# KhaledSharif/yolo-from-scratch

Hardware: NVIDIA B200
Metric: decode+global-NMS + CIoU-loss fwd+bwd throughput @640^2 bs64 nc1 (higher is better)
Workload: dtype f32

## Files before the change

yolo-from-scratch_b200/csrc/yb_nms_graph.cu:

```cuda
#include "yb_common.cuh"
#include "yb_sort.cuh"
#include <cuda_fp16.h>
#include <atomic>
#include <mutex>
#include <vector>

namespace yb {

constexpr int kTile = 32;
constexpr int kSub = 8;
constexpr int kSubs = kTile / kSub;
constexpr uint32_t kNoSub = 0xffffffffu;
constexpr int kGatherThreads = 256;
constexpr int kEdgeThreads = 256;
#ifndef YB_EDGE_CTAS
#define YB_EDGE_CTAS 4
#endif
constexpr int kEdgeCtasPerSM = YB_EDGE_CTAS;
constexpr int kResolveThreads = 1024;

enum { G_PLAIN = 0, G_TRICK = 1, G_CLASS = 2 };

struct GImg {
    int M, mode, exact, overflow;
    int n_tiles;
    u32 n_edges;
    float s_off, t2;
    unsigned long long n_evals;
    unsigned long long n_cands;
};

struct GArgs {
    const float4* boxes;
    const float* scores;
    const int64_t* classes;
    const int* counts;
    int B, cap, tcap, scap;
    float thr;
    int thr_fast_ok;
    float t3;
    u32 k16x2;
    int hexp;
    long long trick_max_numel;
    u32 *k0, *v0;
    int n_score_chunks;
    u32* order;
    u32* rinv;
    u32* pos;
    float4* sboxes;
    u32* skey;
    u32* scls;
    int* iflags;
    int n_chunks;
    u32 resolve_smem_words;
    float4* tstat;
    float4* sstat;
    GImg* info;
    u32* ticket;
    u32 ticket_init;
    uint2* edges;
    u64 edges_per_img;
    int64_t* keep;
    int* n_keep;
};

template <int NT>
__device__ __forceinline__ float block_reduce_minmax(float v, bool is_max, float* s32, int lane, int warp) {
#pragma unroll
    for (int o = 16; o > 0; o >>= 1) {
        const float n = __shfl_xor_sync(0xffffffffu, v, o);
        v = is_max ? fmaxf(v, n) : fminf(v, n);
    }
    __syncthreads();
    if (lane == 0) s32[warp] = v;
    __syncthreads();
    float r = s32[0];
    for (int w = 1; w < NT / 32; ++w) r = is_max ? fmaxf(r, s32[w]) : fminf(r, s32[w]);
    return r;
}

__device__ __forceinline__ unsigned short hilbert_lut_entry(int state, u32 x, u32 y) {
    if (state & 1) { x = 15u - x; y = 15u - y; }
    if (state & 2) { const u32 t = x; x = y; y = t; }
    u32 d = 0, c = 0, sw = 0;
#pragma unroll
    for (u32 s = 8u; s > 0u; s >>= 1) {
        const u32 rx = (x & s) ? 1u : 0u, ry = (y & s) ? 1u : 0u;
        d += s * s * ((3u * rx) ^ ry);
        if (ry == 0u) {
            if (rx == 1u) { x = 15u - x; y = 15u - y; c ^= 1u; }
            const u32 t = x; x = y; y = t;
            sw ^= 1u;
        }
    }
    return (unsigned short)(d | ((((u32)state & 1u) ^ c) << 8) | (((((u32)state >> 1) & 1u) ^ sw) << 9));
}
__device__ __forceinline__ u32 hilbert8(const unsigned short* lut, u32 x, u32 y) {
    const u32 e = lut[((x >> 4) << 4) | (y >> 4)];
    const u32 e2 = lut[((e >> 8) << 8) | ((x & 15u) << 4) | (y & 15u)];
    return ((e & 255u) << 8) | (e2 & 255u);
}

__device__ __forceinline__ u32 area_bucket(const float4 q) {
    const float area = (q.z - q.x) * (q.w - q.y);
    const float lg = fminf(fmaxf(__log2f(area), -44.0f), 120.0f);
    return (u32)(int)floorf(lg * 0.6666667f + 32.0f) & 0x7fu;
}

constexpr int kKeyBits = 14;
struct KeyBits {
    int cls_shift, bkt_shift, bkt_drop, curve_drop;
    u32 bmin;
// ... 52 lines not shown
    const u32* ckey = a.k0 + off;
    const u32 key = ckey[p];
    const int c = p / kScoreChunk;
    u32 rank = (u32)(p - c * kScoreChunk);
    for (int o = 0; o * kScoreChunk < M; ++o) {
        if (o == c) continue;
        const u32* run = ckey + (size_t)o * kScoreChunk;
        const int len = min(kScoreChunk, M - o * kScoreChunk);
        int lo = 0, hi = len;
        while (lo < hi) {
            const int mid = (lo + hi) >> 1;
            const u32 k = run[mid];
            const bool before = o < c ? k <= key : k < key;
            if (before) lo = mid + 1; else hi = mid;
        }
        rank += (u32)lo;
    }
    const u32 idx = a.v0[off + p];
    a.order[off + rank] = idx;
    a.rinv[off + idx] = rank;
}

constexpr int kChunk = 26880;
constexpr int kSpThreads = 1024;
constexpr int kSpBatch = 4;

__host__ __device__ inline size_t spatial_smem_bytes(int ccap) {
    return ((size_t)1 << kKeyBits) * sizeof(u32) + 2 * (((size_t)ccap + 7) / 8 * 8) * sizeof(unsigned short) +
           1024 * sizeof(unsigned short);
}

__global__ void __launch_bounds__(kSpThreads) graph_spatial_kernel(const GArgs a) {
    extern __shared__ __align__(16) u32 s_dyn[];
    __shared__ float s_f[32];
    __shared__ int s_flag[32];
    __shared__ int s_maxcls[32];
    __shared__ int s_bmin[32], s_bmax[32];
    __shared__ u32 s_scan[32];
    constexpr int NT = kSpThreads;
    constexpr int NB = 1 << kKeyBits;

    const int chunk = blockIdx.x, b = blockIdx.y, tid = threadIdx.x, lane = tid & 31, warp = tid >> 5;
    const size_t off = (size_t)b * a.cap;
    {
        const int ccap0 = (min(a.cap, kChunk) + 7) & ~7;
        unsigned short* lut0 = reinterpret_cast<unsigned short*>(s_dyn + NB) + 2 * ccap0;
        lut0[tid] = hilbert_lut_entry(tid >> 8, (u32)(tid >> 4) & 15u, (u32)tid & 15u);
#pragma unroll
        for (int k = 0; k < NB / NT; ++k) s_dyn[k * NT + tid] = 0u;
    }
    int M = a.counts ? a.counts[b] : a.cap;
    M = M < 0 ? 0 : (M > a.cap ? a.cap : M);
    GImg* info = a.info + b;
    if (b == 0 && chunk == 0 && tid == 0) *a.ticket = a.ticket_init;
    const int c0 = chunk * kChunk;
    const int Mc = min(M - c0, kChunk);
    if (Mc <= 0) {
        if (tid == 0 && chunk == 0) {
            GImg z = {0, G_PLAIN, 0, 0, 0, 0u, 0.0f, -1.0f, 0ull, 0ull};
            *info = z;
            if (a.n_chunks == 1) a.iflags[b] = 0;
        }
        return;
    }
    const float4* boxes = a.boxes + off + c0;
    const int64_t* classes = a.classes ? a.classes + off + c0 : nullptr;
    const int ccap = (min(a.cap, kChunk) + 7) & ~7;
    u32* hist = s_dyn;
    unsigned short* keys = reinterpret_cast<unsigned short*>(s_dyn + NB);
    unsigned short* oidx = keys + ccap;
    unsigned short* lut = oidx + ccap;


    const int mode = !a.classes ? G_PLAIN : ((long long)M * 4 <= a.trick_max_numel ? G_TRICK : G_CLASS);
    float mx = -INFINITY, cmin = INFINITY, cmax = -INFINITY;
    int bad = 0, maxcls = 0, bmin = 127, bmax = 0;
    for (int i0 = tid; i0 < Mc; i0 += kSpBatch * NT) {
        float4 qv[kSpBatch];
        long long cv[kSpBatch];
#pragma unroll
        for (int u = 0; u < kSpBatch; ++u) {
            const int i = i0 + u * NT;
            if (i < Mc) {
                qv[u] = __ldg(boxes + i);
                cv[u] = classes ? __ldg(classes + i) : 0ll;
            }
        }
#pragma unroll
        for (int u = 0; u < kSpBatch; ++u) {
            if (i0 + u * NT >= Mc) break;
            const float4 q = qv[u];
            mx = fmaxf(mx, fmaxf(fmaxf(q.x, q.y), fmaxf(q.z, q.w)));
            const bool nan = (q.x != q.x) || (q.y != q.y) || (q.z != q.z) || (q.w != q.w);
            const float big = fmaxf(fmaxf(fabsf(q.x), fabsf(q.y)), fmaxf(fabsf(q.z), fabsf(q.w)));
            bad |= (nan ? 4 : 0) | ((nan || !(big <= 1e17f) || !(q.z >= q.x) || !(q.w >= q.y)) ? 1 : 0);
            const float cx = (q.x + q.z) * 0.5f, cy = (q.y + q.w) * 0.5f;
            cmin = fminf(cmin, fminf(cx, cy));
            cmax = fmaxf(cmax, fmaxf(cx, cy));
            const int bk = (int)area_bucket(q);
            bmin = min(bmin, bk);
            bmax = max(bmax, bk);
            if (classes) {
                const long long c = cv[u];
                bad |= (c < 0 || c >= 512) ? 2 : 0;
                maxcls = max(maxcls, (int)(c & 0x1ff));
            }
        }
// ... 127 lines not shown
    if (p >= M && p < ((M + kSub - 1) & ~(kSub - 1)))
        sbo[p] = make_float4(1e18f, 1e18f, 2e18f, 2e18f);
    if (p < M) {
        const u32 idx = a.pos[off + p];
        float4 q = boxes[idx];
        const float sc = a.scores[off + idx];
        u32 c = 0;
        if (classes) c = (u32)classes[idx];
        if (info.mode == G_TRICK) {
            const float o = (float)classes[idx] * info.s_off;
            q.x += o; q.y += o; q.z += o; q.w += o;
        }
        const u32 cls = (info.mode == G_CLASS) ? c : 0u;
        sbo[p] = q;
        a.skey[off + p] = desc_key(sc);
        if (info.mode == G_CLASS) a.scls[off + p] = cls;
        x1 = f2ord(q.x); y1 = f2ord(q.y); x2 = f2ord(q.z); y2 = f2ord(q.w);
        amin = amax = f2ord((q.z - q.x) * (q.w - q.y));
        c0 = c1 = cls;
    }
    u32 sx1 = x1, sy1 = y1, sx2 = x2, sy2 = y2, samin = amin, samax = amax;
#pragma unroll
    for (int o = 1; o < kSub; o <<= 1) {
        sx1 = min(sx1, __shfl_xor_sync(0xffffffffu, sx1, o));
        sy1 = min(sy1, __shfl_xor_sync(0xffffffffu, sy1, o));
        sx2 = max(sx2, __shfl_xor_sync(0xffffffffu, sx2, o));
        sy2 = max(sy2, __shfl_xor_sync(0xffffffffu, sy2, o));
        samin = min(samin, __shfl_xor_sync(0xffffffffu, samin, o));
        samax = max(samax, __shfl_xor_sync(0xffffffffu, samax, o));
    }
    if ((lane & (kSub - 1)) == 0) {
        float4* ss = a.sstat + (((size_t)b * a.tcap + t) * kSubs + (lane / kSub)) * 2;
        ss[0] = make_float4(ord2f(sx1), ord2f(sy1), ord2f(sx2), ord2f(sy2));
        ss[1] = make_float4(ord2f(samin), ord2f(samax), 0.0f, 0.0f);
    }
    const u32 tx1 = __reduce_min_sync(0xffffffffu, sx1), ty1 = __reduce_min_sync(0xffffffffu, sy1);
    const u32 tx2 = __reduce_max_sync(0xffffffffu, sx2), ty2 = __reduce_max_sync(0xffffffffu, sy2);
    const u32 tamin = __reduce_min_sync(0xffffffffu, samin), tamax = __reduce_max_sync(0xffffffffu, samax);
    c0 = __reduce_min_sync(0xffffffffu, c0);
    c1 = __reduce_max_sync(0xffffffffu, c1);
    if (lane == 0) {
        float4* ts = a.tstat + ((size_t)b * a.tcap + t) * 2;
        ts[0] = make_float4(ord2f(tx1), ord2f(ty1), ord2f(tx2), ord2f(ty2));
        ts[1] = make_float4(ord2f(tamin), ord2f(tamax), __uint_as_float(c0), __uint_as_float(c1));
    }
}

struct Rec16 {
    uint4 box;
    u32 area;
    u32 pad[3];
};
constexpr int kSlots = 8;
constexpr int kQueue = kTile + 8;
constexpr int kCand = 3 * kTile;
constexpr int kItems = kSlots * kTile + kSlots;
struct EdgeWarp {
    Rec16 row16[kTile + 1];
    Rec16 col16[kSlots * 4];
    u32 tl[kTile];
    u32 sub[kQueue];
    uint2 sbx[kQueue];
    u32 sar[kQueue];
    unsigned short irow[kItems];
    unsigned short icol[kItems];
    u32 cand[kCand];
    uint2 ebuf[2 * kTile];
};

__device__ __forceinline__ u32 pack2(const unsigned short lo, const unsigned short hi) { return (u32)lo | ((u32)hi << 16); }
__device__ __forceinline__ __half2 as_h2(const u32 v) { return *reinterpret_cast<const __half2*>(&v); }
__device__ __forceinline__ u32 as_u32(const __half2 v) { return *reinterpret_cast<const u32*>(&v); }
__device__ __forceinline__ unsigned short h_dn(const float v) { return __half_as_ushort(__float2half_rd(v)); }
__device__ __forceinline__ unsigned short h_up(const float v) { return __half_as_ushort(__float2half_ru(v)); }
__device__ __forceinline__ unsigned short h_rz(const float v) { return __half_as_ushort(__float2half_rz(v)); }
__device__ __forceinline__ bool h2_all_ge(const u32 a, const u32 b) {
    u32 r;
    asm("{\n\t.reg .pred p, q;\n\tsetp.ge.f16x2 p|q, %1, %2;\n\tand.pred p, p, q;\n\tselp.u32 %0, 1, 0, p;\n\t}" : "=r"(r) : "r"(a), "r"(b));
    return r != 0u;
}
__device__ __forceinline__ bool h2_any_ge0(const u32 a) {
    u32 r;
    asm("{\n\t.reg .pred p, q;\n\tsetp.ge.f16x2 p|q, %1, %2;\n\tor.pred p, p, q;\n\tselp.u32 %0, 1, 0, p;\n\t}" : "=r"(r) : "r"(a), "r"(0u));
    return r != 0u;
}
__device__ __forceinline__ u32 h2_ge0_bits(const u32 a) {
    u32 r;
    asm("{\n\t.reg .pred p, q;\n\t.reg .u32 t;\n\tsetp.ge.f16x2 p|q, %1, %2;\n\tselp.u32 %0, 1, 0, p;\n\tselp.u32 t, 2, 0, q;\n\tor.b32 %0, %0, t;\n\t}"
        : "=r"(r) : "r"(a), "r"(0u));
    return r;
}

struct Frame {
    float S, S2, nox, noy;
};
__device__ __forceinline__ unsigned short area16_down(const float4 q, const float S2) {
    const float a = __fmul_rd(__fmul_rd(__fsub_rd(q.z, q.x), __fsub_rd(q.w, q.y)), S2);
    return a >= 2.44140625e-4f ? h_rz(fminf(a, 32768.0f)) : (unsigned short)0xfb53u;
}

__device__ __forceinline__ void edge_flush(const GArgs& a, EdgeWarp& w, int b, uint2* __restrict__ edges, int& n_buf) {
    if (n_buf == 0) return;
    const int lane = threadIdx.x & 31;
    __syncwarp();
    u32 base = 0;
    if (lane == 0) base = atomicAdd(&a.info[b].n_edges, (u32)n_buf);
    base = __shfl_sync(0xffffffffu, base, 0);
    for (int k = lane; k < n_buf; k += 32) {
        const u64 idx = (u64)base + k;
        if (idx < a.edges_per_img) edges[idx] = w.ebuf[k];
    }
    __syncwarp();
    n_buf = 0;
// ... 100 lines not shown
                const int at = n_items + __popc(m & lt_mask);
                w.irow[at] = my_row;
                w.icol[at] = (unsigned short)(s * 4 * (int)sizeof(Rec16));
            }
            n_items += __popc(m);
        }
    }
    if (lane < kSlots) {
        w.irow[n_items + lane] = (unsigned short)(kTile * (int)sizeof(Rec16));
        w.icol[n_items + lane] = 0;
    }
    n_evals += (u32)n_items;
    __syncwarp();

    const __half2 K = as_h2(a.k16x2);
    const __half2 zero = as_h2(0u);
    const char* rowbase = reinterpret_cast<const char*>(w.row16);
    const char* colbase = reinterpret_cast<const char*>(w.col16) + j * sizeof(Rec16);
    const unsigned short* irow = w.irow + grp;
    const unsigned short* icol = w.icol + grp;
    for (int it = 0; it < n_items; it += kSlots) {
        const u32 ro = irow[it], co = icol[it];
        const Rec16* rr = reinterpret_cast<const Rec16*>(rowbase + ro);
        const Rec16* cc = reinterpret_cast<const Rec16*>(colbase + co);
        const uint4 R = rr->box, C = cc->box;
        const __half2 iw = __hmax2(__hsub2(__hmin2(as_h2(R.z), as_h2(C.z)), __hmax2(as_h2(R.x), as_h2(C.x))), zero);
        const __half2 ih = __hsub2(__hmin2(as_h2(R.w), as_h2(C.w)), __hmax2(as_h2(R.y), as_h2(C.y)));
        const __half2 sum = __hadd2(as_h2(rr->area), as_h2(cc->area));
        const u32 x = as_u32(__hfma2(__hmul2(iw, ih), K, __hneg2(sum)));
        if (!__any_sync(0xffffffffu, h2_any_ge0(x))) continue;
        const u32 i = ro / (u32)sizeof(Rec16);
        const u32 qp = sub[co / (u32)(4 * sizeof(Rec16))] * kSub + 2 * j;
        const u32 rp = (u32)I * kTile + i;
        u32 hit = ro < (u32)(kTile * sizeof(Rec16)) ? h2_ge0_bits(x) : 0u;
        if (qp <= rp) hit &= 2u;
        if (qp + 1u <= rp) hit = 0u;
        const unsigned m0 = __ballot_sync(0xffffffffu, hit != 0u);
        if (m0 == 0u) continue;
        if (hit) w.cand[n_cand + __popc(m0 & lt_mask)] = (i << 24) | (qp + (hit == 2u ? 1u : 0u));
        n_cand += __popc(m0);
        const unsigned m1 = __ballot_sync(0xffffffffu, hit == 3u);
        if (m1) {
            if (hit == 3u) w.cand[n_cand + __popc(m1 & lt_mask)] = (i << 24) | (qp + 1u);
            n_cand += __popc(m1);
        }
        if (n_cand >= kTile) {
            n_cands += (u32)n_cand;
            cand_process(a, w, M, class_mode, b, I, n_cand, n_buf);
        }
    }
    __syncwarp();
}

__global__ void __launch_bounds__(kEdgeThreads, kEdgeCtasPerSM) graph_edge_kernel(const GArgs a) {
    __shared__ __align__(16) EdgeWarp s_w[kEdgeThreads / 32];
    const int lane = threadIdx.x & 31;
    EdgeWarp& w = s_w[threadIdx.x >> 5];
    const unsigned lt_mask = (1u << lane) - 1u;
    int max_tiles = 0;
    for (int i = lane; i < a.B; i += 32) max_tiles = max(max_tiles, a.iflags[i] ? 0 : a.info[i].n_tiles);
    max_tiles = __reduce_max_sync(0xffffffffu, max_tiles);
    const u32 total = (u32)max_tiles * (u32)a.B;

    bool first = true;
    for (;;) {
        u32 ticket = blockIdx.x * (kEdgeThreads / 32) + (threadIdx.x >> 5);
        if (!first) {
            if (lane == 0) ticket = atomicAdd(a.ticket, 1u);
            ticket = __shfl_sync(0xffffffffu, ticket, 0);
        }
        first = false;
        if (ticket >= total) break;
        const int I = max_tiles - 1 - (int)(ticket / (u32)a.B), b = (int)(ticket % (u32)a.B);
        const float4* sb = a.sboxes + (size_t)b * a.scap;
        const float4* ts = a.tstat + (size_t)b * a.tcap * 2;
        const float4* ss = a.sstat + (size_t)b * a.tcap * kSubs * 2;
        const float4 ib = ts[I * 2], ia = ts[I * 2 + 1];
        const int rp = I * kTile + lane;
        const float4 rq = rp < a.scap ? sb[rp] : make_float4(0.f, 0.f, 0.f, 0.f);
        const int flagged = a.iflags[b];
        const GImg info = a.info[b];
        if (I >= info.n_tiles || flagged) continue;
        const int M = info.M;
        const float t2 = info.t2;
        const float t3 = a.t3;
        const bool class_mode = info.mode == G_CLASS;

        Frame f;
        {
            const float ext = fmaxf(ib.z - ib.x, ib.w - ib.y) * 0.5f;
            int k = a.hexp - ((int)((__float_as_uint(ext) >> 23) & 255u) - 127);
            k = max(-60, min(60, k));
            f.S = __int_as_float((127 + k) << 23);
            f.S2 = f.S * f.S;
            f.nox = -((ib.x + ib.z) * 0.5f) * f.S;
            f.noy = -((ib.y + ib.w) * 0.5f) * f.S;
        }
        const u32 icmin = __float_as_uint(ia.z), icmax = __float_as_uint(ia.w);

        const bool rvalid = rp < M;
        u32 r_lo = 0x63d063d0u, r_hi = 0xe3d0e3d0u, r_wh_t = 0x63d063d0u, r_ar = 0xe3d063d0u;
        __syncwarp();
        {
            Rec16& r16 = w.row16[lane];
            uint4 box = make_uint4(0x63d063d0u, 0x63d063d0u, 0xe3d0e3d0u, 0xe3d0e3d0u);
            u32 area = 0x3c003c00u;
            if (rvalid) {
                const unsigned short x1 = h_dn(__fmaf_rd(rq.x, f.S, f.nox)), y1 = h_dn(__fmaf_rd(rq.y, f.S, f.noy));
                const unsigned short x2 = h_up(__fmaf_ru(rq.z, f.S, f.nox)), y2 = h_up(__fmaf_ru(rq.w, f.S, f.noy));
                const unsigned short ar = area16_down(rq, f.S2);
                const float wd = __fsub_rd(rq.z, rq.x), hd = __fsub_rd(rq.w, rq.y);
                const unsigned short wt = h_rz(__fmul_rd(__fmul_rd(wd, f.S), t3)), ht = h_rz(__fmul_rd(__fmul_rd(hd, f.S), t3));
                const unsigned short at = h_rz(__fmul_rd(__fmul_rd(__fmul_rd(wd, hd), f.S2), t3));
                const unsigned short au = h_up(__fmul_ru(__fmul_ru(__fsub_ru(rq.z, rq.x), __fsub_ru(rq.w, rq.y)), f.S2)) ^ 0x8000u;
                r_lo = pack2(x1, y1);
                r_hi = pack2(x2, y2);
                r_wh_t = pack2(wt, ht);
                r_ar = pack2(at, au);
                box = make_uint4(pack2(x1, x1), pack2(y1, y1), pack2(x2, x2), pack2(y2, y2));
                area = pack2(ar, ar);
            }
            r16.box = box;
            r16.area = area;
            if (lane == 0) {
                Rec16& sen = w.row16[kTile];
                sen.box = make_uint4(0x63d063d0u, 0x63d063d0u, 0xe3d0e3d0u, 0xe3d0e3d0u);
                sen.area = 0x3c003c00u;
            }
        }
        __syncwarp();
        u32 n_evals = 0, n_cands = 0;
        int n_q = 0;
        int n_buf = 0;
        int n_cand = 0;

        constexpr int kCT = kChunk / kTile;
        int chunk_end = min(info.n_tiles, (I / kCT + 1) * kCT);
        for (int J0 = I;; J0 += 32) {
            if (J0 >= chunk_end && chunk_end < info.n_tiles) {
                J0 = chunk_end;
                chunk_end = min(info.n_tiles, chunk_end + kCT);
                if (class_mode) {
                    const int step = (chunk_end - J0 + 31) / 32;
                    const int Jp = J0 + lane * step;
                    const bool ge = Jp < chunk_end && __float_as_uint(ts[Jp * 2 + 1].w) >= icmin;
                    const unsigned m = __ballot_sync(0xffffffffu, ge);
                    const int first = m ? __ffs(m) - 1 : 32;
                    J0 += max(first - 1, 0) * step;
                }
            }
            const bool tail = J0 >= info.n_tiles;
            int n_t = 0;
            int n_tail = kSlots;
            if (tail) {
                if (n_q == 0) break;
                if (lane >= n_q && lane < kSlots) w.sub[lane] = kNoSub;
                n_tail = n_q;
                n_q = kSlots;
                __syncwarp();
            } else {
                const int Jl = J0 + lane;
                bool ok = Jl < chunk_end;
                float4 jb = make_float4(0.f, 0.f, 0.f, 0.f), ja = jb;
                if (ok) { jb = ts[Jl * 2]; ja = ts[Jl * 2 + 1]; }
                if (class_mode) {
                    const bool beyond = !ok || __float_as_uint(ja.z) > icmax;
                    ok = ok && !beyond && __float_as_uint(ja.w) >= icmin;
                    if (__ballot_sync(0xffffffffu, beyond) == 0xffffffffu) {
                        J0 = chunk_end - 32;
                        continue;
                    }
                }
                if (ok) {
                    ok = fminf(ib.z, jb.z) > fmaxf(ib.x, jb.x) && fminf(ib.w, jb.w) > fmaxf(ib.y, jb.y) &&
                         ia.y >= t2 * ja.x && ja.y >= t2 * ia.x;
                }
                const unsigned cand = __ballot_sync(0xffffffffu, ok);
                if (cand == 0u) continue;
                if (ok) w.tl[__popc(cand & lt_mask)] = (u32)Jl;
                __syncwarp();
                n_t = __popc(cand);
            }
            int t0 = 0;
            do {
                if (t0 < n_t) {
                    const int k = t0 + lane / kSubs;
                    bool sok = k < n_t;
                    u32 e = 0u;
                    float4 sbx = make_float4(0.f, 0.f, 0.f, 0.f), sar = sbx;
                    if (sok) {
                        e = w.tl[k] * kSubs + (u32)(lane & (kSubs - 1));
                        sok = (int)(e * kSub) < M;
                        if (sok) {
                            sbx = ss[e * 2]; sar = ss[e * 2 + 1];
                            sok = fminf(ib.z, sbx.z) > fmaxf(ib.x, sbx.x) && fminf(ib.w, sbx.w) > fmaxf(ib.y, sbx.y) &&
                                  ia.y >= t2 * sar.x && sar.y >= t2 * ia.x;
                        }
                    }
                    const unsigned sm = __ballot_sync(0xffffffffu, sok);
                    if (sok) {
                        const int qi = n_q + __popc(sm & lt_mask);
                        w.sub[qi] = e;
                        w.sbx[qi] = make_uint2(pack2(h_dn(__fmaf_rd(sbx.x, f.S, f.nox)), h_dn(__fmaf_rd(sbx.y, f.S, f.noy))),
                                               pack2(h_up(__fmaf_ru(sbx.z, f.S, f.nox)), h_up(__fmaf_ru(sbx.w, f.S, f.noy))));
                        const unsigned short amax = h_up(__fmul_ru(__fmul_ru(sar.y, 1.0000077f), f.S2));
                        const unsigned short amin = h_rz(__fmul_rd(__fmul_rd(__fmul_rd(sar.x, 0.9999923f), f.S2), t3));
                        w.sar[qi] = pack2(amax, amin ^ 0x8000u);
                    }
                    n_q += __popc(sm);
                    __syncwarp();
                }
                int head = 0;
                if (n_tail == kSlots) {
                    for (; n_q - head >= kSlots; head += kSlots)
                        edge_chunk<true>(a, w, M, class_mode, b, I, head, sb, f, kSlots, r_lo, r_hi, r_wh_t, r_ar, n_evals,
                                         n_cands, n_cand, n_buf);
                } else {
                    edge_chunk<false>(a, w, M, class_mode, b, I, 0, sb, f, n_tail, r_lo, r_hi, r_wh_t, r_ar, n_evals, n_cands,
                                      n_cand, n_buf);
                    head = kSlots;
                }
                if (head) {
                    const int rem = n_q - head;
                    u32 v = 0u, va = 0u;
                    uint2 vb = make_uint2(0u, 0u);
                    if (lane < rem) { v = w.sub[head + lane]; vb = w.sbx[head + lane]; va = w.sar[head + lane]; }
                    __syncwarp();
                    if (lane < rem) { w.sub[lane] = v; w.sbx[lane] = vb; w.sar[lane] = va; }
                    __syncwarp();
                    n_q = rem;
                }
                t0 += 32 / kSubs;
            } while (t0 < n_t);
        }
        if (n_cand) {
            n_cands += (u32)n_cand;
            cand_process(a, w, M, class_mode, b, I, n_cand, n_buf);
        }
        edge_flush(a, w, b, a.edges + (u64)b * a.edges_per_img, n_buf);
        if (lane == 0 && n_evals) {
            atomicAdd(&a.info[b].n_evals, (unsigned long long)n_evals);
            atomicAdd(&a.info[b].n_cands, (unsigned long long)n_cands);
        }
    }
}

constexpr int kGreedyT = 512;
struct GreedySmem {
    float4 blk[kGreedyT];
    float4 kt[kGreedyT];
    long long bcls[kGreedyT];
    long long kcls[kGreedyT];
    u32 mask[kGreedyT * (kGreedyT / 32)];
    u32 dead[kGreedyT / 32];
    u32 keptbits[kGreedyT / 32];
    u32 K;
};

__device__ __forceinline__ bool iou_gt_exact(const float4 a, const float4 b, const float thr) {
    const float left = fmaxf(a.x, b.x), right = fminf(a.z, b.z);
    const float top = fmaxf(a.y, b.y), bottom = fminf(a.w, b.w);
    const float w = fmaxf(right - left, 0.0f), h = fmaxf(bottom - top, 0.0f);
    const float inter = w * h;
    const float sa = (a.z - a.x) * (a.w - a.y);
    const float den = __fmaf_rn(b.z - b.x, b.w - b.y, sa) - inter;
    return (inter / den) > thr;
}

__device__ void greedy_resolve(const GArgs& a, const GImg& info, int b, GreedySmem& g) {
    const int tid = threadIdx.x, lane = tid & 31, warp = tid >> 5;
    const int i = tid & (kGreedyT - 1), h = tid / kGreedyT;
    const int M = info.M;
    const size_t off = (size_t)b * a.cap;
    const float4* boxes = a.boxes + off;
    const int64_t* classes = a.classes ? a.classes + off : nullptr;
    const u32* __restrict__ order = a.order + off;
    int64_t* keep = a.keep + off;
    const float thr = a.thr;
    const bool trick = info.mode == G_TRICK, per_class = info.mode == G_CLASS;
    const float far = 3.0e38f;
    constexpr int W = kGreedyT / 32, HALF = kGreedyT / 2;
    if (tid == 0) g.K = 0u;
    __syncthreads();
    for (int r0 = 0; r0 < M; r0 += kGreedyT) {
        const int n = min(kGreedyT, M - r0);
        if (tid < kGreedyT) {
// ... 178 lines not shown
            const u32 kept = u & ~fK[w] & ~fU[w];
            const u32 nu = u & ~(sup | kept);
            U[w] = nu;
            K[w] |= kept;
            fK[w] = 0u; fU[w] = 0u;
            left |= nu != 0u;
        }
        if (!__syncthreads_or(left)) break;
    }
    const u32* __restrict__ order = a.order + (size_t)b * a.cap;
    int64_t* __restrict__ keep = a.keep + (size_t)b * a.cap;
    const int chunk = (nw + kResolveThreads - 1) / kResolveThreads;
    const int c0 = min(tid * chunk, nw), c1 = min(c0 + chunk, nw);
    u32 sum = 0;
    for (int w = c0; w < c1; ++w) sum += __popc(K[w]);
    u32 inc = sum;
#pragma unroll
    for (int o = 1; o < 32; o <<= 1) {
        const u32 n = __shfl_up_sync(0xffffffffu, inc, o);
        if (lane >= o) inc += n;
    }
    if (lane == 31) s_scan[warp] = inc;
    __syncthreads();
    u32 base = inc - sum, total = 0;
    for (int w = 0; w < 32; ++w) {
        if (w < warp) base += s_scan[w];
        total += s_scan[w];
    }
    for (int w = c0; w < c1; ++w) {
        fK[w] = base;
        base += __popc(K[w]);
    }
    __syncthreads();
    for (int r0 = tid; r0 < M; r0 += 4 * kResolveThreads) {
        u32 idx[4];
#pragma unroll
        for (int k = 0; k < 4; ++k) {
            const int r = r0 + k * kResolveThreads;
            idx[k] = r < M ? order[r] : 0u;
        }
#pragma unroll
        for (int k = 0; k < 4; ++k) {
            const int r = r0 + k * kResolveThreads;
            if (r < M) {
                const u32 bits = K[r >> 5];
                if ((bits >> (r & 31)) & 1u) keep[fK[r >> 5] + __popc(bits & ((1u << (r & 31)) - 1u))] = (int64_t)idx[k];
            }
        }
    }
    if (tid == 0) a.n_keep[b] = (int)total;
}

struct GLayout {
    size_t k[2], order, rinv, pos, sboxes, skey, scls, tstat, sstat, info, iflags, ticket, edges, total;
};

static inline size_t g_align(size_t x) { return (x + 255) / 256 * 256; }

static GLayout graph_layout(int B, int cap) {
    GLayout L;
    size_t o = 0;
    const size_t n = (size_t)B * cap;
    const size_t tcap = ((size_t)cap + kTile - 1) / kTile;
    const size_t nk = cap > kS16MaxM ? n : 0;
    for (int i = 0; i < 2; ++i) { L.k[i] = o; o = g_align(o + nk * 4); }
    L.order = o; o = g_align(o + n * 4);
    L.rinv = o; o = g_align(o + n * 4);
    L.pos = o; o = g_align(o + n * 4);
    L.sboxes = o; o = g_align(o + (size_t)B * (((size_t)cap + kSub - 1) / kSub * kSub) * 16);
    L.skey = o; o = g_align(o + n * 4);
    L.scls = o; o = g_align(o + n * 4);
    L.tstat = o; o = g_align(o + (size_t)B * tcap * 32);
    L.sstat = o; o = g_align(o + (size_t)B * tcap * kSubs * 32);
    L.info = o; o = g_align(o + (size_t)B * sizeof(GImg));
    L.iflags = o; o = g_align(o + (size_t)B * sizeof(int));
    L.ticket = o; o = g_align(o + 256);
    L.edges = o;
    L.total = o;
    return L;
}

size_t graph_min_workspace(int B, int cap) { return graph_layout(B, cap).total + (size_t)B * 8; }

struct ForkJoin {
    cudaStream_t side = nullptr;
    static constexpr int kRing = 32;
    cudaEvent_t fork[kRing] = {}, join[kRing] = {};
    std::atomic<unsigned> next{0};
    bool ok = false;
};
static ForkJoin* fork_join_for_device() {
    static std::mutex mu;
    static ForkJoin* per_dev[64] = {};
    int dev = 0;
    if (cudaGetDevice(&dev) != cudaSuccess || dev < 0 || dev >= 64) return nullptr;
    std::lock_guard<std::mutex> lk(mu);
    if (!per_dev[dev]) {
        ForkJoin* f = new ForkJoin();
        bool ok = cudaStreamCreateWithFlags(&f->side, cudaStreamNonBlocking) == cudaSuccess;
        for (int i = 0; ok && i < ForkJoin::kRing; ++i)
            ok = cudaEventCreateWithFlags(&f->fork[i], cudaEventDisableTiming) == cudaSuccess &&
                 cudaEventCreateWithFlags(&f->join[i], cudaEventDisableTiming) == cudaSuccess;
        f->ok = ok;
        if (!ok) cudaGetLastError();
        per_dev[dev] = f;
    }
    return per_dev[dev]->ok ? per_dev[dev] : nullptr;
}

int graph_nms(const float* boxes, const float* scores, const int64_t* classes, const int* counts, int B, int cap,
              double iou_threshold, long long trick_max_numel, int64_t* keep, int* n_keep, void* ws,
              size_t ws_bytes, cudaStream_t st) {
    GLayout L = graph_layout(B, cap);
    YB_CHECK_ARG(ws_bytes >= L.total + (size_t)B * 8, "nms(graph): workspace too small (%zu < %zu)", ws_bytes,
                 L.total + (size_t)B * 8);
    char* w = reinterpret_cast<char*>(ws);
    GArgs a;
    a.boxes = reinterpret_cast<const float4*>(boxes); a.scores = scores; a.classes = classes; a.counts = counts;
    a.B = B; a.cap = cap; a.tcap = (cap + kTile - 1) / kTile; a.scap = (cap + kSub - 1) / kSub * kSub;
    a.n_chunks = (cap + kChunk - 1) / kChunk;
    a.thr = (float)iou_threshold;
    a.thr_fast_ok = (a.thr >= 0.03f && a.thr <= 1e30f) ? 1 : 0;
    a.t3 = a.thr * (1.0f - 0.015625f);
    {
        const double th = (double)a.thr * (1.0 - 1.0 / 4096.0);
        const double K = a.thr_fast_ok ? (1.0 + th) / th * (1.0 + 1.0 / 64.0) * (1.0 + 1.0 / 512.0) : 1.0;
        const unsigned short kb = __half_as_ushort(__float2half_rn((float)K));
        a.k16x2 = (u32)kb | ((u32)kb << 16);
        a.hexp = a.thr >= 0.35f ? 5 : (a.thr >= 0.1f ? 4 : 3);
    }
    a.trick_max_numel = trick_max_numel;
    a.k0 = (u32*)(w + L.k[0]); a.v0 = (u32*)(w + L.k[1]);
    a.n_score_chunks = (cap + kScoreChunk - 1) / kScoreChunk;
    a.order = (u32*)(w + L.order); a.rinv = (u32*)(w + L.rinv); a.pos = (u32*)(w + L.pos);
    a.sboxes = (float4*)(w + L.sboxes); a.skey = (u32*)(w + L.skey); a.scls = (u32*)(w + L.scls);
    a.tstat = (float4*)(w + L.tstat);
    a.sstat = (float4*)(w + L.sstat);
    a.info = (GImg*)(w + L.info);
    a.iflags = (int*)(w + L.iflags);
    a.ticket = (u32*)(w + L.ticket);
    a.ticket_init = (u32)(sm_count() * kEdgeCtasPerSM * (kEdgeThreads / 32));
    a.edges = (uint2*)(w + L.edges);
    a.edges_per_img = (ws_bytes - L.edges) / 8 / (size_t)B;
    a.keep = keep; a.n_keep = n_keep;

    ForkJoin* fj = fork_join_for_device();
    cudaStream_t ss = st;
    int slot = 0;
    if (fj) {
        slot = (int)(fj->next.fetch_add(1u) % ForkJoin::kRing);
        YB_CUDA(cudaEventRecord(fj->fork[slot], st));
        YB_CUDA(cudaStreamWaitEvent(fj->side, fj->fork[slot], 0));
        ss = fj->side;
    }
    {
        const size_t sort_smem = s16_smem_bytes(cap < kScoreChunk ? cap : kScoreChunk);
        YB_CUDA(cudaFuncSetAttribute(graph_score_kernel, cudaFuncAttributeMaxDynamicSharedMemorySize, (int)sort_smem));
        YB_LAUNCH("graph_score_kernel", ss,
                  (graph_score_kernel<<<dim3(a.n_score_chunks, B), kS16Threads, sort_smem, ss>>>(a)));
        if (a.n_score_chunks > 1)
            YB_LAUNCH("graph_score_merge_kernel", ss,
                      (graph_score_merge_kernel<<<dim3((cap + 255) / 256, B), 256, 0, ss>>>(a)));
    }
    if (fj) YB_CUDA(cudaEventRecord(fj->join[slot], fj->side));

    if (a.n_chunks > 1) YB_CUDA(cudaMemsetAsync(a.iflags, 0, (size_t)B * sizeof(int), st));
    {
        const size_t smem = spatial_smem_bytes(cap < kChunk ? cap : kChunk);
        YB_CUDA(cudaFuncSetAttribute(graph_spatial_kernel, cudaFuncAttributeMaxDynamicSharedMemorySize, (int)smem));
        YB_LAUNCH("graph_spatial_kernel", st, graph_spatial_kernel<<<dim3(a.n_chunks, B), kSpThreads, smem, st>>>(a));
    }
    const dim3 ggrid((a.tcap + kGatherThreads / 32 - 1) / (kGatherThreads / 32), B);
    YB_LAUNCH("graph_gather_kernel", st, graph_gather_kernel<<<ggrid, kGatherThreads, 0, st>>>(a));
    const int ctas = sm_count() * kEdgeCtasPerSM;
    YB_LAUNCH("graph_edge_kernel", st, graph_edge_kernel<<<ctas, kEdgeThreads, 0, st>>>(a));

    if (fj) YB_CUDA(cudaStreamWaitEvent(st, fj->join[slot], 0));
    static_assert(kResolveThreads == 2 * kGreedyT, "greedy_resolve splits the CTA in two halves");
    const size_t bits_bytes = ((size_t)((cap + 31) / 32) * 4 + 2) * 4;
    YB_CHECK_ARG(bits_bytes <= 150 * 1024, "nms(graph): cap too large for the resolve kernel");
    size_t dyn = 160 * 1024;
    a.resolve_smem_words = (u32)((dyn - bits_bytes) / 4);
    if (dyn < sizeof(GreedySmem)) dyn = sizeof(GreedySmem);
    YB_CUDA(cudaFuncSetAttribute(graph_resolve_kernel, cudaFuncAttributeMaxDynamicSharedMemorySize, (int)dyn));
    YB_LAUNCH("graph_resolve_kernel", st, graph_resolve_kernel<<<B, kResolveThreads, dyn, st>>>(a));
    return 0;
}

int graph_stats(const void* ws, size_t ws_bytes, int B, int cap, unsigned long long* evals, unsigned long long* edges,
                unsigned long long* cands, cudaStream_t st) {
    GLayout L = graph_layout(B, cap);
    YB_CHECK_ARG(ws && ws_bytes >= L.total, "nms_graph_stats: not a graph workspace");
    std::vector<GImg> h((size_t)B);
    YB_CUDA(cudaMemcpyAsync(h.data(), reinterpret_cast<const char*>(ws) + L.info, (size_t)B * sizeof(GImg),
                            cudaMemcpyDeviceToHost, st));
    YB_CUDA(cudaStreamSynchronize(st));
    unsigned long long ev = 0, ed = 0, ca = 0;
    for (auto& g : h) { ev += g.n_evals * (unsigned long long)kSub; ed += g.n_edges; ca += g.n_cands; }
    if (evals) *evals = ev;
    if (edges) *edges = ed;
    if (cands) *cands = ca;
    return 0;
}

}
```

Measured before the change: 228,800.

## Split NMS edge work into a tile-pair cull pass and fixed-size work items

```diff
diff --git a/yolo-from-scratch_b200/csrc/yb_nms_graph.cu b/yolo-from-scratch_b200/csrc/yb_nms_graph.cu
--- a/yolo-from-scratch_b200/csrc/yb_nms_graph.cu
+++ b/yolo-from-scratch_b200/csrc/yb_nms_graph.cu
@@ -14,9 +14,13 @@
 constexpr int kGatherThreads = 256;
 constexpr int kEdgeThreads = 256;
 #ifndef YB_EDGE_CTAS
-#define YB_EDGE_CTAS 4
+#define YB_EDGE_CTAS 5
 #endif
 constexpr int kEdgeCtasPerSM = YB_EDGE_CTAS;
+constexpr int kCullThreads = 256;
+constexpr int kCullSteps = 4;
+constexpr int kItemTiles = 8;
+constexpr int kItemBudget = 16;
 constexpr int kResolveThreads = 1024;
 
 enum { G_PLAIN = 0, G_TRICK = 1, G_CLASS = 2 };
@@ -58,6 +62,11 @@
     GImg* info;
     u32* ticket;
     u32 ticket_init;
+    u32* item_count;
+    uint2* items;
+    unsigned short* tlist;
+    u32 item_cap;
+    int cull_steps;
     uint2* edges;
     u64 edges_per_img;
     int64_t* keep;
@@ -216,7 +225,10 @@
     int M = a.counts ? a.counts[b] : a.cap;
     M = M < 0 ? 0 : (M > a.cap ? a.cap : M);
     GImg* info = a.info + b;
-    if (b == 0 && chunk == 0 && tid == 0) *a.ticket = a.ticket_init;
+    if (b == 0 && chunk == 0 && tid == 0) {
+        *a.ticket = a.ticket_init;
+        *a.item_count = 0u;
+    }
     const int c0 = chunk * kChunk;
     const int Mc = min(M - c0, kChunk);
     if (Mc <= 0) {
@@ -450,13 +462,13 @@
     u32 pad[3];
 };
 constexpr int kSlots = 8;
-constexpr int kQueue = kTile + 8;
+constexpr int kQueue = kItemTiles * kSubs;
 constexpr int kCand = 3 * kTile;
 constexpr int kItems = kSlots * kTile + kSlots;
+static_assert(kQueue == 32, "level 2 of a work item is one step: lane <-> (tile, sub-tile)");
 struct EdgeWarp {
     Rec16 row16[kTile + 1];
     Rec16 col16[kSlots * 4];
-    u32 tl[kTile];
     u32 sub[kQueue];
     uint2 sbx[kQueue];
     u32 sar[kQueue];
@@ -663,15 +675,99 @@
     __syncwarp();
 }
 
+__global__ void __launch_bounds__(kCullThreads) graph_cull_kernel(const GArgs a) {
+    extern __shared__ uint2 s_steps[];
+    const int b = blockIdx.y, lane = threadIdx.x & 31, warp = threadIdx.x >> 5;
+    const unsigned lt_mask = (1u << lane) - 1u;
+    const int I = blockIdx.x * (kCullThreads / 32) + warp;
+    const GImg info = a.info[b];
+    if (I >= info.n_tiles || a.iflags[b]) return;
+    uint2* steps = s_steps + (size_t)warp * a.cull_steps;
+    const float4* ts = a.tstat + (size_t)b * a.tcap * 2;
+    const float4 ib = ts[I * 2], ia = ts[I * 2 + 1];
+    const float t2 = info.t2;
+    const bool class_mode = info.mode == G_CLASS;
+    const u32 icmin = __float_as_uint(ia.z), icmax = __float_as_uint(ia.w);
+
+    constexpr int kCT = kChunk / kTile;
+    int n_steps = 0, n = 0;
+    int chunk_end = min(info.n_tiles, (I / kCT + 1) * kCT);
+    for (int J0 = I;;) {
+        if (J0 >= chunk_end && chunk_end < info.n_tiles) {
+            J0 = chunk_end;
+            chunk_end = min(info.n_tiles, chunk_end + kCT);
+            if (class_mode) {
+                const int step = (chunk_end - J0 + 31) / 32;
+                const int Jp = J0 + lane * step;
+                const bool ge = Jp < chunk_end && __float_as_uint(ts[Jp * 2 + 1].w) >= icmin;
+                const unsigned m = __ballot_sync(0xffffffffu, ge);
+                const int first = m ? __ffs(m) - 1 : 32;
+                J0 += max(first - 1, 0) * step;
+            }
+        }
+        if (J0 >= info.n_tiles) break;
+        float4 jb[kCullSteps], ja[kCullSteps];
+#pragma unroll
+        for (int u = 0; u < kCullSteps; ++u) {
+            const int Jl = J0 + 32 * u + lane;
+            jb[u] = ja[u] = make_float4(0.f, 0.f, 0.f, 0.f);
+            if (Jl < chunk_end) { jb[u] = ts[Jl * 2]; ja[u] = ts[Jl * 2 + 1]; }
+        }
+        int next = J0 + 32 * kCullSteps;
+#pragma unroll
+        for (int u = 0; u < kCullSteps; ++u) {
+            const int Ju = J0 + 32 * u;
+            if (Ju >= chunk_end) { next = Ju; break; }
+            const int Jl = Ju + lane;
+            bool ok = Jl < chunk_end;
+            if (class_mode) {
+                const bool beyond = !ok || __float_as_uint(ja[u].z) > icmax;
+                ok = ok && !beyond && __float_as_uint(ja[u].w) >= icmin;
+                if (__ballot_sync(0xffffffffu, beyond) == 0xffffffffu) { next = chunk_end; break; }
+            }
+            if (ok) {
+                ok = fminf(ib.z, jb[u].z) > fmaxf(ib.x, jb[u].x) && fminf(ib.w, jb[u].w) > fmaxf(ib.y, jb[u].y) &&
+                     ia.y >= t2 * ja[u].x && ja[u].y >= t2 * ia.x;
+            }
+            const unsigned cand = __ballot_sync(0xffffffffu, ok);
+            if (cand) {
+                if (lane == 0) steps[n_steps] = make_uint2((u32)Ju, cand);
+                ++n_steps;
+                n += __popc(cand);
+            }
+        }
+        J0 = next;
+    }
+    if (n == 0) return;
+    const u32 n_items = (u32)(n + kItemTiles - 1) / kItemTiles;
+    u32 base = 0;
+    if (lane == 0) {
+        base = atomicAdd(a.item_count, n_items);
+        if (base + n_items > a.item_cap) atomicOr(a.iflags + b, 8);
+    }
+    base = __shfl_sync(0xffffffffu, base, 0);
+    __syncwarp();
+    for (u32 k = lane; k < n_items; k += 32)
+        if (base + k < a.item_cap)
+            a.items[base + k] = make_uint2((u32)b, ((u32)I << 4) | (u32)min(kItemTiles, n - (int)k * kItemTiles));
+    int pre = 0;
+    for (int s = 0; s < n_steps; ++s) {
+        const uint2 st = steps[s];
+        if ((st.y >> lane) & 1u) {
+            const u32 idx = (u32)pre + __popc(st.y & lt_mask);
+            if (base + idx / kItemTiles < a.item_cap)
+                a.tlist[(size_t)base * kItemTiles + idx] = (unsigned short)(st.x + lane);
+        }
+        pre += __popc(st.y);
+    }
+}
+
 __global__ void __launch_bounds__(kEdgeThreads, kEdgeCtasPerSM) graph_edge_kernel(const GArgs a) {
     __shared__ __align__(16) EdgeWarp s_w[kEdgeThreads / 32];
     const int lane = threadIdx.x & 31;
     EdgeWarp& w = s_w[threadIdx.x >> 5];
     const unsigned lt_mask = (1u << lane) - 1u;
-    int max_tiles = 0;
-    for (int i = lane; i < a.B; i += 32) max_tiles = max(max_tiles, a.iflags[i] ? 0 : a.info[i].n_tiles);
-    max_tiles = __reduce_max_sync(0xffffffffu, max_tiles);
-    const u32 total = (u32)max_tiles * (u32)a.B;
+    const u32 total = min(*a.item_count, a.item_cap);
 
     bool first = true;
     for (;;) {
@@ -682,16 +778,23 @@
         }
         first = false;
         if (ticket >= total) break;
-        const int I = max_tiles - 1 - (int)(ticket / (u32)a.B), b = (int)(ticket % (u32)a.B);
+        const uint2 item = a.items[ticket];
+        const int k = lane / kSubs;
+        const u32 J = a.tlist[(size_t)ticket * kItemTiles + k];
+        const int b = (int)item.x, I = (int)(item.y >> 4), n_t = (int)(item.y & 15u);
         const float4* sb = a.sboxes + (size_t)b * a.scap;
         const float4* ts = a.tstat + (size_t)b * a.tcap * 2;
         const float4* ss = a.sstat + (size_t)b * a.tcap * kSubs * 2;
         const float4 ib = ts[I * 2], ia = ts[I * 2 + 1];
         const int rp = I * kTile + lane;
         const float4 rq = rp < a.scap ? sb[rp] : make_float4(0.f, 0.f, 0.f, 0.f);
+        const u32 e = J * kSubs + (u32)(lane & (kSubs - 1));
+        const bool sin = k < n_t;
+        float4 sbx = make_float4(0.f, 0.f, 0.f, 0.f), sar = sbx;
+        if (sin) { sbx = ss[e * 2]; sar = ss[e * 2 + 1]; }
         const int flagged = a.iflags[b];
         const GImg info = a.info[b];
-        if (I >= info.n_tiles || flagged) continue;
+        if (flagged) continue;
         const int M = info.M;
         const float t2 = info.t2;
         const float t3 = a.t3;
@@ -700,14 +803,13 @@
         Frame f;
         {
             const float ext = fmaxf(ib.z - ib.x, ib.w - ib.y) * 0.5f;
-            int k = a.hexp - ((int)((__float_as_uint(ext) >> 23) & 255u) - 127);
-            k = max(-60, min(60, k));
-            f.S = __int_as_float((127 + k) << 23);
+            int kx = a.hexp - ((int)((__float_as_uint(ext) >> 23) & 255u) - 127);
+            kx = max(-60, min(60, kx));
+            f.S = __int_as_float((127 + kx) << 23);
             f.S2 = f.S * f.S;
             f.nox = -((ib.x + ib.z) * 0.5f) * f.S;
             f.noy = -((ib.y + ib.w) * 0.5f) * f.S;
         }
-        const u32 icmin = __float_as_uint(ia.z), icmax = __float_as_uint(ia.w);
 
         const bool rvalid = rp < M;
         u32 r_lo = 0x63d063d0u, r_hi = 0xe3d0e3d0u, r_wh_t = 0x63d063d0u, r_ar = 0xe3d063d0u;
@@ -739,110 +841,35 @@
                 sen.area = 0x3c003c00u;
             }
         }
+
+        const bool sok = sin && (int)(e * kSub) < M &&
+                         fminf(ib.z, sbx.z) > fmaxf(ib.x, sbx.x) && fminf(ib.w, sbx.w) > fmaxf(ib.y, sbx.y) &&
+                         ia.y >= t2 * sar.x && sar.y >= t2 * ia.x;
+        const unsigned sm = __ballot_sync(0xffffffffu, sok);
+        if (sok) {
+            const int qi = __popc(sm & lt_mask);
+            w.sub[qi] = e;
+            w.sbx[qi] = make_uint2(pack2(h_dn(__fmaf_rd(sbx.x, f.S, f.nox)), h_dn(__fmaf_rd(sbx.y, f.S, f.noy))),
+                                   pack2(h_up(__fmaf_ru(sbx.z, f.S, f.nox)), h_up(__fmaf_ru(sbx.w, f.S, f.noy))));
+            const unsigned short amax = h_up(__fmul_ru(__fmul_ru(sar.y, 1.0000077f), f.S2));
+            const unsigned short amin = h_rz(__fmul_rd(__fmul_rd(__fmul_rd(sar.x, 0.9999923f), f.S2), t3));
+            w.sar[qi] = pack2(amax, amin ^ 0x8000u);
+        }
+        const int n_q = __popc(sm);
         __syncwarp();
+
         u32 n_evals = 0, n_cands = 0;
-        int n_q = 0;
         int n_buf = 0;
         int n_cand = 0;
-
-        constexpr int kCT = kChunk / kTile;
-        int chunk_end = min(info.n_tiles, (I / kCT + 1) * kCT);
-        for (int J0 = I;; J0 += 32) {
-            if (J0 >= chunk_end && chunk_end < info.n_tiles) {
-                J0 = chunk_end;
-                chunk_end = min(info.n_tiles, chunk_end + kCT);
-                if (class_mode) {
-                    const int step = (chunk_end - J0 + 31) / 32;
-                    const int Jp = J0 + lane * step;
-                    const bool ge = Jp < chunk_end && __float_as_uint(ts[Jp * 2 + 1].w) >= icmin;
-                    const unsigned m = __ballot_sync(0xffffffffu, ge);
-                    const int first = m ? __ffs(m) - 1 : 32;
-                    J0 += max(first - 1, 0) * step;
-                }
-            }
-            const bool tail = J0 >= info.n_tiles;
-            int n_t = 0;
-            int n_tail = kSlots;
-            if (tail) {
-                if (n_q == 0) break;
-                if (lane >= n_q && lane < kSlots) w.sub[lane] = kNoSub;
-                n_tail = n_q;
-                n_q = kSlots;
-                __syncwarp();
-            } else {
-                const int Jl = J0 + lane;
-                bool ok = Jl < chunk_end;
-                float4 jb = make_float4(0.f, 0.f, 0.f, 0.f), ja = jb;
-                if (ok) { jb = ts[Jl * 2]; ja = ts[Jl * 2 + 1]; }
-                if (class_mode) {
-                    const bool beyond = !ok || __float_as_uint(ja.z) > icmax;
-                    ok = ok && !beyond && __float_as_uint(ja.w) >= icmin;
-                    if (__ballot_sync(0xffffffffu, beyond) == 0xffffffffu) {
-                        J0 = chunk_end - 32;
-                        continue;
-                    }
-                }
-                if (ok) {
-                    ok = fminf(ib.z, jb.z) > fmaxf(ib.x, jb.x) && fminf(ib.w, jb.w) > fmaxf(ib.y, jb.y) &&
-                         ia.y >= t2 * ja.x && ja.y >= t2 * ia.x;
-                }
-                const unsigned cand = __ballot_sync(0xffffffffu, ok);
-                if (cand == 0u) continue;
-                if (ok) w.tl[__popc(cand & lt_mask)] = (u32)Jl;
-                __syncwarp();
-                n_t = __popc(cand);
-            }
-            int t0 = 0;
-            do {
-                if (t0 < n_t) {
-                    const int k = t0 + lane / kSubs;
-                    bool sok = k < n_t;
-                    u32 e = 0u;
-                    float4 sbx = make_float4(0.f, 0.f, 0.f, 0.f), sar = sbx;
-                    if (sok) {
-                        e = w.tl[k] * kSubs + (u32)(lane & (kSubs - 1));
-                        sok = (int)(e * kSub) < M;
-                        if (sok) {
-                            sbx = ss[e * 2]; sar = ss[e * 2 + 1];
-                            sok = fminf(ib.z, sbx.z) > fmaxf(ib.x, sbx.x) && fminf(ib.w, sbx.w) > fmaxf(ib.y, sbx.y) &&
-                                  ia.y >= t2 * sar.x && sar.y >= t2 * ia.x;
-                        }
-                    }
-                    const unsigned sm = __ballot_sync(0xffffffffu, sok);
-                    if (sok) {
-                        const int qi = n_q + __popc(sm & lt_mask);
-                        w.sub[qi] = e;
-                        w.sbx[qi] = make_uint2(pack2(h_dn(__fmaf_rd(sbx.x, f.S, f.nox)), h_dn(__fmaf_rd(sbx.y, f.S, f.noy))),
-                                               pack2(h_up(__fmaf_ru(sbx.z, f.S, f.nox)), h_up(__fmaf_ru(sbx.w, f.S, f.noy))));
-                        const unsigned short amax = h_up(__fmul_ru(__fmul_ru(sar.y, 1.0000077f), f.S2));
-                        const unsigned short amin = h_rz(__fmul_rd(__fmul_rd(__fmul_rd(sar.x, 0.9999923f), f.S2), t3));
-                        w.sar[qi] = pack2(amax, amin ^ 0x8000u);
-                    }
-                    n_q += __popc(sm);
-                    __syncwarp();
-                }
-                int head = 0;
-                if (n_tail == kSlots) {
-                    for (; n_q - head >= kSlots; head += kSlots)
-                        edge_chunk<true>(a, w, M, class_mode, b, I, head, sb, f, kSlots, r_lo, r_hi, r_wh_t, r_ar, n_evals,
-                                         n_cands, n_cand, n_buf);
-                } else {
-                    edge_chunk<false>(a, w, M, class_mode, b, I, 0, sb, f, n_tail, r_lo, r_hi, r_wh_t, r_ar, n_evals, n_cands,
-                                      n_cand, n_buf);
-                    head = kSlots;
-                }
-                if (head) {
-                    const int rem = n_q - head;
-                    u32 v = 0u, va = 0u;
-                    uint2 vb = make_uint2(0u, 0u);
-                    if (lane < rem) { v = w.sub[head + lane]; vb = w.sbx[head + lane]; va = w.sar[head + lane]; }
-                    __syncwarp();
-                    if (lane < rem) { w.sub[lane] = v; w.sbx[lane] = vb; w.sar[lane] = va; }
-                    __syncwarp();
-                    n_q = rem;
-                }
-                t0 += 32 / kSubs;
-            } while (t0 < n_t);
+        int head = 0;
+        for (; n_q - head >= kSlots; head += kSlots)
+            edge_chunk<true>(a, w, M, class_mode, b, I, head, sb, f, kSlots, r_lo, r_hi, r_wh_t, r_ar, n_evals, n_cands,
+                             n_cand, n_buf);
+        if (head < n_q) {
+            if (lane >= n_q - head && lane < kSlots) w.sub[head + lane] = kNoSub;
+            __syncwarp();
+            edge_chunk<false>(a, w, M, class_mode, b, I, head, sb, f, n_q - head, r_lo, r_hi, r_wh_t, r_ar, n_evals,
+                              n_cands, n_cand, n_buf);
         }
         if (n_cand) {
             n_cands += (u32)n_cand;
@@ -1127,10 +1154,18 @@
 }
 
 struct GLayout {
-    size_t k[2], order, rinv, pos, sboxes, skey, scls, tstat, sstat, info, iflags, ticket, edges, total;
+    size_t k[2], order, rinv, pos, sboxes, skey, scls, tstat, sstat, info, iflags, ticket, items, tlist, edges, total;
+    u32 item_cap;
 };
 
 static inline size_t g_align(size_t x) { return (x + 255) / 256 * 256; }
+
+static size_t item_capacity(int B, size_t tcap) {
+    const size_t q = tcap / kItemTiles, r = tcap % kItemTiles;
+    const size_t worst = kItemTiles * q * (q + 1) / 2 + r * (q + 1);
+    const size_t budget = (size_t)kItemBudget * tcap;
+    return (size_t)B * (worst < budget ? worst : budget);
+}
 
 static GLayout graph_layout(int B, int cap) {
     GLayout L;
@@ -1150,6 +1185,10 @@
     L.info = o; o = g_align(o + (size_t)B * sizeof(GImg));
     L.iflags = o; o = g_align(o + (size_t)B * sizeof(int));
     L.ticket = o; o = g_align(o + 256);
+    const size_t items = item_capacity(B, tcap);
+    L.item_cap = (u32)items;
+    L.items = o; o = g_align(o + items * sizeof(uint2));
+    L.tlist = o; o = g_align(o + items * kItemTiles * sizeof(unsigned short));
     L.edges = o;
     L.total = o;
     return L;
@@ -1186,6 +1225,8 @@
 int graph_nms(const float* boxes, const float* scores, const int64_t* classes, const int* counts, int B, int cap,
               double iou_threshold, long long trick_max_numel, int64_t* keep, int* n_keep, void* ws,
               size_t ws_bytes, cudaStream_t st) {
+    const size_t bits_bytes = ((size_t)((cap + 31) / 32) * 4 + 2) * 4;
+    YB_CHECK_ARG(bits_bytes <= 150 * 1024, "nms(graph): cap too large for the resolve kernel");
     GLayout L = graph_layout(B, cap);
     YB_CHECK_ARG(ws_bytes >= L.total + (size_t)B * 8, "nms(graph): workspace too small (%zu < %zu)", ws_bytes,
                  L.total + (size_t)B * 8);
@@ -1215,6 +1256,11 @@
     a.iflags = (int*)(w + L.iflags);
     a.ticket = (u32*)(w + L.ticket);
     a.ticket_init = (u32)(sm_count() * kEdgeCtasPerSM * (kEdgeThreads / 32));
+    a.item_count = a.ticket + 1;
+    a.items = (uint2*)(w + L.items);
+    a.tlist = (unsigned short*)(w + L.tlist);
+    a.item_cap = L.item_cap;
+    a.cull_steps = a.n_chunks * ((kChunk / kTile + 31) / 32);
     a.edges = (uint2*)(w + L.edges);
     a.edges_per_img = (ws_bytes - L.edges) / 8 / (size_t)B;
     a.keep = keep; a.n_keep = n_keep;
@@ -1247,13 +1293,16 @@
     }
     const dim3 ggrid((a.tcap + kGatherThreads / 32 - 1) / (kGatherThreads / 32), B);
     YB_LAUNCH("graph_gather_kernel", st, graph_gather_kernel<<<ggrid, kGatherThreads, 0, st>>>(a));
+    {
+        const dim3 cgrid((a.tcap + kCullThreads / 32 - 1) / (kCullThreads / 32), B);
+        const size_t smem = (size_t)(kCullThreads / 32) * a.cull_steps * sizeof(uint2);
+        YB_LAUNCH("graph_cull_kernel", st, graph_cull_kernel<<<cgrid, kCullThreads, smem, st>>>(a));
+    }
     const int ctas = sm_count() * kEdgeCtasPerSM;
     YB_LAUNCH("graph_edge_kernel", st, graph_edge_kernel<<<ctas, kEdgeThreads, 0, st>>>(a));
 
     if (fj) YB_CUDA(cudaStreamWaitEvent(st, fj->join[slot], 0));
     static_assert(kResolveThreads == 2 * kGreedyT, "greedy_resolve splits the CTA in two halves");
-    const size_t bits_bytes = ((size_t)((cap + 31) / 32) * 4 + 2) * 4;
-    YB_CHECK_ARG(bits_bytes <= 150 * 1024, "nms(graph): cap too large for the resolve kernel");
     size_t dyn = 160 * 1024;
     a.resolve_smem_words = (u32)((dyn - bits_bytes) / 4);
     if (dyn < sizeof(GreedySmem)) dyn = sizeof(GreedySmem);
```

Result: slower. 213,700 (median of 6 runs) (-6.6%).
